# RoboSafe-Lab/Controllable-Latent-Diffusion-for-Traffic-Simulation

Measured on AMD Instinct MI355X. Metric: denoising-step·agent/s, higher is better.
Workload: dtype f32; 1 GPU; BASELINE configs[2]: 32 scenes x 64 agents per GPU, 100 denoising steps (DDPM ancestral loop of the reference), latent seq 52 x 4, cond 256, CFG w=2.0 (2 U-Net passes per step, non_cond_feat); target-speed guidance gradient through decoder + roll-out on every step t > 0; + LSTM decode + unicycle roll-out; scenes_total=32, agents_this_rank=2048, agents_total=2048, denoise_steps=100, guidance_gradient=True, sim_steps_per_bench_step=0, weights=random init (synth seed 0)

## Files before the change

### controllable-latent-diffusion-for-traffic-simulation_amd/csrc/cld_api.hip

```cpp
#include <hip/hip_runtime.h>

#include <cmath>
#include <cstdio>
#include <cstdlib>
#include <cstring>
#include <map>
#include <string>
#include <vector>

#include "../../include/cld.h"
#include "cld_kernels.h"
#include "train.h"

using namespace cld;

namespace {

constexpr int T = 52, D = 4, COND = 256, TE = 32, NCB = 1792, ACT = 3328;
constexpr int NBUF = 8;

struct ConvLayer {
    ConvGeom g{};
    bool has_a = false, has_b = false;
    float *wfrag = nullptr, *bias = nullptr, *gamma = nullptr, *beta = nullptr;
// ... 241 lines not shown
        static const char* th = getenv("CLD_TILING_HALF");
#else
        constexpr const char* th = nullptr;
#endif
        const long wgs_b = (long)(b_pad / (MT / l.g.lm)) * (l.c_out / 32);
        int best = 0;
        double best_cost = 1e30;
        for (int hm = 0; hm <= 3; ++hm) {
            ConvGeom tg = *g; tg.half = hm;
            if (!conv_geom_supported(tg)) continue;
            if (th && th[0] != '0' + hm && (th[0] == '0' || th[0] == '1' || th[0] == '2' || th[0] == '3')) continue;
            const long n = wgs_b << hm, rounds = (n + 255) / 256;
            const int nmt = ((208 >> hm) + 15) / 16;
            double cost = (double)rounds * nmt / (rounds == 1 ? 0.85 : 0.92);
            if (l.g.stride == 2 && hm == 0) cost *= 1.15;
            if (cost < best_cost * (b_pad >= 1024 ? 0.97 : 1.0)) { best_cost = cost; best = hm; }
        }
        if (cost_c <= best_cost) return set(32, 4, 2);
        g->half = best;
        if (best == 3 && (wgs_b << 3) * roles <= 256 && c1c2_mult_of_64(l)) {
            ConvGeom d = *g; d.kc = 64; d.nwn = 2; d.ks = 4;
            if (conv_geom_supported(d)) return set(64, 2, 4);
        }
        return true;
    }
    return false;
}

struct Ws {
    float *xw, *xtmp, *meanb, *cb, *buf[NBUF], *guide;
    float *gcur, *adam_m, *adam_v;
    float *col_traj, *col_grad;
    float* col_act;
};
size_t ws_floats(int b_pad) {
    return (size_t)b_pad * (3 * T * D + NCB + (size_t)NBUF * ACT) + guide_scratch_floats(b_pad) + (size_t)b_pad * (3 * T * D + 2 * T * 6 + T * 2);
}
Ws carve(void* ws, int b_pad) {
    Ws w;
    float* p = static_cast<float*>(ws);
    w.xw = p; p += (size_t)b_pad * T * D;
    w.xtmp = p; p += (size_t)b_pad * T * D;
    w.meanb = p; p += (size_t)b_pad * T * D;
    w.cb = p; p += (size_t)b_pad * NCB;
    for (int i = 0; i < NBUF; ++i) { w.buf[i] = p; p += (size_t)b_pad * ACT; }
    w.guide = p; p += guide_scratch_floats(b_pad);
    w.gcur = p; p += (size_t)b_pad * T * D;
    w.adam_m = p; p += (size_t)b_pad * T * D;
    w.adam_v = p; p += (size_t)b_pad * T * D;
    w.col_traj = p; p += (size_t)b_pad * T * 6;
    w.col_grad = p; p += (size_t)b_pad * T * 6;
    w.col_act = p;
    return w;
}
inline int pad16(int b) { return (b + 15) / 16 * 16; }

ConvArgs make_args(cld_handle h, const ConvLayer& l, const float* x1, const float* x2, float* y, const float* res,
                   const float* cb, const float* tb_row) {
    ConvArgs a{};
    a.x1 = x1; a.x2 = x2; a.c1_real = l.c1_real; a.c1_pad = l.c1_pad; a.c2 = l.c2;
    a.wfrag = l.wfrag; a.bias = l.bias; a.gamma = l.gamma; a.beta = l.beta;
    if (l.cb_off >= 0) { a.cbias = cb + l.cb_off; a.cb_stride = NCB; a.tbias = tb_row ? tb_row + l.cb_off : nullptr; }
    a.res = res; a.y = y; a.c_out = l.c_out; a.ly = l.ly; a.off0 = l.off0; a.orow0 = l.orow0;
    a.wscale_inv = l.g.ain == 1 ? 1.0f / kWScale : 1.0f;
    a.stamps = nullptr;
    (void)h;
    return a;
}

constexpr int kWino1dMinRows = 384;
bool conv5_takes_winograd(int l_in, int c1, int c2, int c_out, long b_pad, int forced) {
    if (!wino1d_supported(l_in, c1, c2, c_out) || forced == CLD_FORM_DIRECT) return false;
    const long widest = c1 > c_out ? c1 : c_out;
    if (b_pad * l_in * widest * 4 >= (1L << 31)) return false;
    return forced == CLD_FORM_WINOGRAD || forced == CLD_FORM_WINOGRAD_WHOLE || forced == CLD_FORM_WINOGRAD_KSPLIT || b_pad >= kWino1dMinRows;
}
int wino_item_form(cld_handle h) {
    const int f = h->force_kernel[CLD_KERNEL_CONV5];
    return f == CLD_FORM_WINOGRAD_WHOLE ? 1 : f == CLD_FORM_WINOGRAD_KSPLIT ? 2 : 0;
}
bool use_wino1d(cld_handle h, const ConvLayer& l, int b_pad) {
    if (!l.ufrag || !l.wino_launch) return false;
    return conv5_takes_winograd(l.g.l_in, l.c1_real, l.c2, l.c_out, b_pad, h->force_kernel[CLD_KERNEL_CONV5]);
}
void count_flop(cld_handle h, const ConvLayer& l, int b_pad, double* alg, double* exec) {
// ... 983 lines not shown
    a.urgency = g->urgency; a.pref_speed = g->pref_speed; a.scale = g->scale; a.reached = g->reached; a.grad_in = grad_in;
    a.loss = loss; a.grad = grad; a.rows = B; a.num_samp = g->num_samp; a.global_t = g->global_t; a.dt = g->dt;
    a.min_progress_dist = g->min_progress_dist;
    return a;
}

static int check_guidance(cld_handle h, const char* fn, const cld_guidance* gd, int B) {
    if (!h->has_decoder) return fail(h, CLD_ERR_STATE, std::string(fn) + ": guidance needs the decoder weights");
    if (!gd->curr_states || (!gd->target_speed && !gd->speed_limit_scale && !gd->acc_limit_scale && !gd->target_pos_scale && !gd->ext_grad && !gd->collision && !gd->map_collision && !h->has_goal))
        return fail(h, CLD_ERR_ARG, std::string(fn) + ": guidance needs curr_states and at least one loss term");
    if (gd->collision) {
        const int rcc = check_collision(h, fn, gd->collision, B);
        if (rcc) return rcc;
    }
    if (gd->map_collision) {
        const int rcc = check_map_collision(h, fn, gd->map_collision, B);
        if (rcc) return rcc;
    }
    if (h->has_goal) {
        const int rcc = check_goal(h, fn, &h->goal, B);
        if (rcc) return rcc;
    }
    if (gd->grad_steps < 0 || gd->final_grad_steps < 0 || gd->grad_steps > 64 || gd->final_grad_steps > 64)
        return fail(h, CLD_ERR_ARG, std::string(fn) + ": grad_steps out of range (0..64)");
    if (gd->optimizer != CLD_GUIDE_ADAM && gd->optimizer != CLD_GUIDE_SGD) return fail(h, CLD_ERR_ARG, std::string(fn) + ": unknown optimizer");
    if (gd->apply_output && gd->final_optimizer != CLD_GUIDE_ADAM && gd->final_optimizer != CLD_GUIDE_SGD)
        return fail(h, CLD_ERR_ARG, std::string(fn) + ": unknown optimizer for the output step");
    if (gd->target_pos_scale && (!gd->target_pos || !gd->target_time)) return fail(h, CLD_ERR_ARG, std::string(fn) + ": target_pos_scale needs target_pos and target_time");
    return CLD_OK;
}

static int run_guidance(cld_handle h, const Ws& w, const cld_guidance* gd, int B, bool intermediate, float sigma_t, float sigma_noise,
                        const float* mean0, const float* cond, const float* z, uint64_t seed, unsigned long long salt,
                        float* mean_out, float* x_out, float* x_out2, float* grad_out, hipStream_t s) {
    GuideArgs g{};
    g.cond = cond; g.curr_states = gd->curr_states; g.target_speed = gd->target_speed; g.loss_scale = gd->loss_scale;
    g.speed_limit_scale = gd->speed_limit_scale; g.acc_limit_scale = gd->acc_limit_scale;
    g.speed_limit = gd->speed_limit; g.acc_limit = gd->acc_limit;
    g.target_pos = gd->target_pos; g.target_time = gd->target_time; g.target_pos_scale = gd->target_pos_scale;
    g.ext_grad = gd->ext_grad;
    const float lr_in = intermediate ? gd->lr : gd->final_lr, th_in = intermediate ? gd->perturb_th : gd->final_perturb_th;
    g.scratch = w.guide; g.lr = lr_in > 0.f ? lr_in : sigma_t; g.perturb_th = th_in > 0.f ? th_in : (th_in == 0.f ? sigma_t : -1.f);
    g.optimizer = intermediate ? gd->optimizer : gd->final_optimizer; g.B = B; g.seed = seed; g.step_salt = salt;
    const int steps_in = intermediate ? gd->grad_steps : gd->final_grad_steps;
    const int steps = steps_in > 1 ? steps_in : 1;
    g.opt_steps = steps; g.mean0 = mean0; g.adam_m = w.adam_m; g.adam_v = w.adam_v;
    for (int k = 1; k <= steps; ++k) {
        const bool last = k == steps;
        g.opt_step = k;
        g.mean = k == 1 ? mean0 : w.gcur;
        if (gd->collision || gd->map_collision || h->has_goal) {
            if (B >= 256 && guide_forward_available(B, h->force_kernel[CLD_KERNEL_GUIDE]) && h->force_kernel[CLD_KERNEL_DECODE] == FORM_AUTO) {
                GuideArgs gf{};
                gf.mean = g.mean; gf.cond = cond; gf.curr_states = gd->curr_states; gf.scratch = w.guide; gf.B = B; gf.act_out = w.col_act;
                HIPCK(h, launch_guide_forward(h->dec, h->dyn, gf, s));
                HIPCK(h, launch_action_to_state(h->dyn, w.col_act, gd->curr_states, w.col_traj, B, 1, 1, s));
                g.act_in = guide_split_available(B, h->force_kernel[CLD_KERNEL_GUIDE]) && h->force_kernel[CLD_KERNEL_GUIDE] == FORM_AUTO ? w.col_act : nullptr;
            } else {
                HIPCK(h, launch_decode(h->dec, h->dyn, g.mean, cond, gd->curr_states, nullptr, w.col_traj, B, 1, s, h->force_kernel[CLD_KERNEL_DECODE]));
            }
        }
        if (gd->collision) {
            const cld_collision* c = gd->collision;
            CollisionArgs ca{};
            ca.traj = w.col_traj; ca.extent = c->extent; ca.world_from_agent = c->world_from_agent; ca.curr_speed = c->curr_speed;
            ca.scene_start = c->scene_start; ca.scene_weight = c->scene_weight; ca.guided = c->guided; ca.excluded = c->excluded; ca.max_scene_agents = c->max_scene_agents; ca.grad_in = gd->ext_grad;
            ca.grad = w.col_grad; ca.B_agents = B / c->num_samp; ca.num_scenes = c->num_scenes; ca.num_samp = c->num_samp;
            ca.num_disks = c->num_disks; ca.buffer_dist = c->buffer_dist; ca.decay_rate = c->decay_rate; ca.moving_speed_th = c->moving_speed_th;
            HIPCK(h, launch_agent_collision(ca, s));
            g.ext_grad = w.col_grad;
        }
        if (gd->map_collision) {
            HIPCK(h, launch_map_collision(map_args(gd->map_collision, w.col_traj, gd->collision ? w.col_grad : gd->ext_grad, nullptr, w.col_grad), B, s));
            g.ext_grad = w.col_grad;
        }
        if (h->has_goal) {
            HIPCK(h, launch_goal(goal_args(&h->goal, w.col_traj, (gd->collision || gd->map_collision) ? w.col_grad : gd->ext_grad, nullptr, w.col_grad, B), s));
            g.ext_grad = w.col_grad;
        }
        g.z = last ? z : nullptr;
        g.sigma = last ? sigma_noise : 0.f;
        g.mean_out = last ? mean_out : w.gcur;
        g.x_out = last ? x_out : nullptr;
        g.x_out2 = last ? x_out2 : nullptr;
        g.grad_out = k == 1 ? grad_out : nullptr;
        HIPCK(h, launch_guide(h->dec, h->dyn, g, s, h->force_kernel[CLD_KERNEL_GUIDE]));
    }
    return CLD_OK;
}

static int sample_iteration(cld_handle h, const Ws& w, bool cfg, int B, int bp, int i, const float* z, uint64_t seed,
                            unsigned long long salt, const float* cond, float guidance_w, const cld_guidance* gd,
                            float* mean_guided, float* grad, bool want_mean, hipStream_t s) {
    const int bpn = cfg ? 2 * bp : bp;
    float* x_hi = w.xw + (size_t)bp * T * D;
    const float sigma = std::exp(0.5f * h->plvc[i]);
    const bool guide = gd && (i > 0 ? !gd->no_intermediate : gd->apply_output != 0);
    HeadArgs a{};
    a.w = h->head_w; a.b = h->head_b; a.x = w.xw; a.B = B; a.b_pad = bp;
    a.z = z;
    a.seed = seed; a.step_salt = salt;
    a.xc = h->x_t_cof[i]; a.nc = h->noise_cof[i];
    a.sg = (i == 0) ? 0.f : sigma;
    if (guide) {
        a.mean_out = w.meanb;
        if (gd->guide_clean) {
            a.xc = h->sqrt_recip_acp[i]; a.nc = h->sqrt_recipm1_acp[i];
        }
    } else {
        a.x_out = w.xw;
        a.x_out2 = cfg ? x_hi : nullptr;
        a.mean_out = (i == 0 || want_mean) ? w.meanb : nullptr;
    }
    h->fuse_upd = cfg ? nullptr : &a;
    const hipError_t eu = run_unet(h, w, w.xw, i, bpn, s);
    h->fuse_upd = nullptr;
    HIPCK(h, eu);
    if (!h->upd_fused) {
        head_source(h, w, a);
        if (cfg) {
            if (a.eps_in) a.eps_in_uncond = a.eps_in + (size_t)bp * T * D;
            else a.f_uncond = w.buf[7] + (size_t)bp * T * 64;
            a.cfg_w = guidance_w;
        }
        HIPCK(h, launch_head(a, s));
    }
    if (guide) {
        int rcg = run_guidance(h, w, gd, B, i > 0, sigma, a.sg, w.meanb, cond, a.z, seed, salt, mean_guided ? mean_guided : (i == 0 ? w.xtmp : nullptr),
                               w.xw, cfg ? x_hi : nullptr, grad, s);
        if (rcg) return rcg;
    }
    return CLD_OK;
}

static int sample_impl(cld_handle h, const char* fn, const float* x_T, const float* noise, const float* cond,
                       const float* non_cond, float guidance_w, const cld_guidance* gd, int32_t steps, float* x0, float* x1,
                       float* logp, int32_t B, uint64_t seed, void* workspace, size_t workspace_bytes, void* stream) {
    const bool cfg = non_cond != nullptr;
    int rc = check_common(h, fn, cfg ? 2 * pad16(B) : B, 0, workspace, workspace_bytes);
    if (rc) return rc;
    if (!x_T || !cond) return fail(h, CLD_ERR_ARG, std::string(fn) + ": null pointer");
    if (steps != loop_steps(h))
        return fail(h, CLD_ERR_ARG, std::string(fn) + ": steps must equal len(range(0, n_timesteps, stride)) = " + std::to_string(loop_steps(h)));
    if (gd && (rc = check_guidance(h, fn, gd, B)) != CLD_OK) return rc;
    hipStream_t s = static_cast<hipStream_t>(stream);
    const int bp = pad16(B), bpn = cfg ? 2 * bp : bp;
    Ws w = carve(workspace, bpn);
    float* x_hi = w.xw + (size_t)bp * T * D;
    HIPCK(h, launch_pack_latent(x_T, w.xw, B, bp, s));
    HIPCK(h, launch_cond_bias(cond, h->wc, h->cbias_b, w.cb, B, bp, NCB, s));
    if (cfg) {
        HIPCK(h, launch_pack_latent(x_T, x_hi, B, bp, s));
        HIPCK(h, launch_cond_bias(non_cond, h->wc, h->cbias_b, w.cb + (size_t)bp * NCB, B, bp, NCB, s));
    }
    for (int it = 0; it < steps; ++it) {
        const int i = (steps - 1 - it) * h->stride;
        rc = sample_iteration(h, w, cfg, B, bp, i, noise ? noise + (size_t)it * B * T * D : nullptr, seed, (unsigned long long)it, cond,
                              guidance_w, gd, nullptr, nullptr, false, s);
        if (rc) return rc;
        if (i == 1 && x1) HIPCK(h, launch_unpack(w.xw, x1, B, s));
        if (i == 0) {
            if (x0) HIPCK(h, launch_unpack(w.xw, x0, B, s));
            if (logp) HIPCK(h, launch_logprob(w.xw, (gd && gd->apply_output) ? w.xtmp : w.meanb, std::exp(0.5f * h->plvc[0]), logp, B, s));
        }
    }
    return CLD_OK;
}

int cld_sample_step(cld_handle h, const float* x_t, const float* cond, const float* non_cond, float guidance_w,
                    const cld_guidance* gd, int32_t t_idx, const float* z, float* x_next, float* mean, float* mean_guided,
                    float* grad, float* sigma_host, int32_t B, void* workspace, size_t workspace_bytes, void* stream) {
    const bool cfg = non_cond != nullptr;
    int rc = check_common(h, "cld_sample_step", cfg ? 2 * pad16(B) : B, t_idx, workspace, workspace_bytes);
    if (rc) return rc;
    if (!x_t || !cond || (!z && t_idx != 0)) return fail(h, CLD_ERR_ARG, "cld_sample_step: null pointer");
    if (gd && (rc = check_guidance(h, "cld_sample_step", gd, B)) != CLD_OK) return rc;
    if (sigma_host) *sigma_host = std::exp(0.5f * h->plvc[t_idx]);
    hipStream_t s = static_cast<hipStream_t>(stream);
    const int bp = pad16(B), bpn = cfg ? 2 * bp : bp;
    Ws w = carve(workspace, bpn);
    HIPCK(h, launch_pack_latent(x_t, w.xw, B, bp, s));
    HIPCK(h, launch_cond_bias(cond, h->wc, h->cbias_b, w.cb, B, bp, NCB, s));
    if (cfg) {
        HIPCK(h, launch_pack_latent(x_t, w.xw + (size_t)bp * T * D, B, bp, s));
        HIPCK(h, launch_cond_bias(non_cond, h->wc, h->cbias_b, w.cb + (size_t)bp * NCB, B, bp, NCB, s));
    }
    rc = sample_iteration(h, w, cfg, B, bp, t_idx, z, 0, 0, cond, guidance_w, gd, mean_guided, grad, mean != nullptr, s);
    if (rc) return rc;
    if (x_next) HIPCK(h, launch_unpack(w.xw, x_next, B, s));
    if (mean) HIPCK(h, launch_unpack(w.meanb, mean, B, s));
    return CLD_OK;
// ... 461 lines not shown
```

### controllable-latent-diffusion-for-traffic-simulation_amd/csrc/cld_kernels.h

```cpp
#pragma once
#include <hip/hip_runtime.h>
#include <stdint.h>

namespace cld {

inline hipError_t set_max_lds_once(const void* fn, int bytes, unsigned long long* done_mask) {
    int dev = 0;
    hipError_t e = hipGetDevice(&dev);
    if (e != hipSuccess) return e;
    if (dev >= 0 && dev < 64 && ((*done_mask >> dev) & 1ull)) return hipSuccess;
    e = hipFuncSetAttribute(fn, hipFuncAttributeMaxDynamicSharedMemorySize, bytes);
    if (e != hipSuccess) return e;
    if (dev >= 0 && dev < 64) *done_mask |= 1ull << dev;
    return hipSuccess;
}

constexpr int MT = 208;
constexpr int NMT = 13;

enum { EPI_BIAS = 0, EPI_GN_MISH = 1 };

struct ConvArgs {
    const float* x1;
    const float* x2;
// ... 203 lines not shown
    const float *c_wt[5], *c_b[5], *c_g[4], *c_be[4];
};
hipError_t launch_context_head(const ContextHeadArgs& a, hipStream_t s);

struct GuideArgs {
    const float* mean;
    const float* cond;
    const float* curr_states;
    const float* target_speed;
    const float* loss_scale;
    const float* speed_limit_scale;
    const float* acc_limit_scale;
    float speed_limit, acc_limit;
    const float* target_pos;
    const int* target_time;
    const float* target_pos_scale;
    const float* ext_grad;
    const float* z;
    float* mean_out;
    float* x_out;
    float* x_out2;
    float* grad_out;
    float* act_out;
    const float* act_in;
    float* scratch;
    float lr, perturb_th, sigma;
    int optimizer;
    int opt_step, opt_steps;
    const float* mean0;
    float* adam_m;
    float* adam_v;
    int B;
    unsigned long long seed, step_salt;
};
size_t guide_scratch_floats(int B);
void read_guide_stamps(unsigned long long* out);
hipError_t launch_guide(const DecoderWeights& w, const DynParams& d, const GuideArgs& a, hipStream_t s, int form = FORM_AUTO);
bool guide_forward_available(int B, int form = FORM_AUTO);
bool guide_split_available(int B, int form = FORM_AUTO);
hipError_t launch_guide_forward(const DecoderWeights& w, const DynParams& d, const GuideArgs& a, hipStream_t s);

hipError_t launch_guide_losses(const GuideArgs& a, const float* traj, float* losses, hipStream_t s);

struct CollisionArgs {
    const float* traj;
    const float* extent;
    const float* world_from_agent;
    const float* curr_speed;
    const int* scene_start;
    const float* scene_weight;
    const unsigned char* guided;
    const unsigned char* excluded;
    const float* grad_in;
    float* loss;
    float* grad;
    int B_agents, num_scenes, num_samp, num_disks;
    int max_scene_agents;
    float buffer_dist, decay_rate, moving_speed_th;
};
hipError_t launch_agent_collision(const CollisionArgs& a, hipStream_t s);

struct MapCollisionArgs {
    const float* traj;
    const float* extent;
    const float* raster_from_agent;
    const unsigned char* drivable_map;
    const float* curr_speed;
    const int* scene_start;
// ... 64 lines not shown
```

### controllable-latent-diffusion-for-traffic-simulation_amd/csrc/guide_kernels.hip

```cpp
#include "cld_kernels.h"

namespace cld {

typedef float v4f __attribute__((ext_vector_type(4)));

__device__ __forceinline__ float sigmoid_g(float x) { return 1.0f / (1.0f + expf(-x)); }

constexpr int GT = 52;
__device__ __forceinline__ void chain_grad(const DynParams& d, const GuideArgs& a, int b, const float* act0, const float* act1, int st,
                                           float* dact0, float* dact1, float* sc) {
    float* vk = sc; float* th = sc + 54; float* gv = sc + 108; float* gth = sc + 162;
    float* gxk = sc + 216; float* gyk = sc + 270;
    const float* cs = a.curr_states + (size_t)b * 4;
    const float* tgt = a.target_speed ? a.target_speed + (size_t)b * GT : nullptr;
    const float s_ts = tgt ? (a.loss_scale ? a.loss_scale[b] : (1.0f / (float)GT)) : 0.f;
    const float s_sl = a.speed_limit_scale ? a.speed_limit_scale[b] : 0.f;
    const float s_al = a.acc_limit_scale ? a.acc_limit_scale[b] : 0.f;
    const float s_tp = a.target_pos_scale ? a.target_pos_scale[b] : 0.f;
    const float* eg = a.ext_grad ? a.ext_grad + (size_t)b * GT * 6 : nullptr;
    const bool pos = s_tp != 0.f || eg != nullptr;
    float v_raw = cs[2], x = cs[0], y = cs[1], yaw = cs[3];
    vk[0] = fminf(fmaxf(v_raw, d.v_lo), d.v_hi);
    th[0] = yaw;
    gv[0] = 0.f;
// ... 969 lines not shown

__device__ __forceinline__ float sum_over_units(float x) {
    x += __builtin_bit_cast(float, __builtin_amdgcn_update_dpp(0, __builtin_bit_cast(int, x), 0x124 , 0xf, 0xf, false));
    x += __builtin_bit_cast(float, __builtin_amdgcn_update_dpp(0, __builtin_bit_cast(int, x), 0x128 , 0xf, 0xf, false));
    const auto r16 = __builtin_amdgcn_permlane16_swap(__builtin_bit_cast(unsigned, x), __builtin_bit_cast(unsigned, x), false, false);
    const unsigned a16 = r16[0], b16 = r16[1];
    x = __builtin_bit_cast(float, a16) + __builtin_bit_cast(float, b16);
    const auto r32 = __builtin_amdgcn_permlane32_swap(__builtin_bit_cast(unsigned, x), __builtin_bit_cast(unsigned, x), false, false);
    const unsigned a32 = r32[0], b32 = r32[1];
    return __builtin_bit_cast(float, a32) + __builtin_bit_cast(float, b32);
}

__device__ __forceinline__ float add_other_half(float x) {
    const auto r32 = __builtin_amdgcn_permlane32_swap(__builtin_bit_cast(unsigned, x), __builtin_bit_cast(unsigned, x), false, false);
    const unsigned a32 = r32[0], b32 = r32[1];
    return __builtin_bit_cast(float, a32) + __builtin_bit_cast(float, b32);
}

__device__ __forceinline__ float quad_xor1(float v) { return __builtin_bit_cast(float, __builtin_amdgcn_update_dpp(0, __builtin_bit_cast(int, v), 0xB1 , 0xf, 0xf, false)); }
__device__ __forceinline__ float quad_xor2(float v) { return __builtin_bit_cast(float, __builtin_amdgcn_update_dpp(0, __builtin_bit_cast(int, v), 0x4E , 0xf, 0xf, false)); }
__device__ __forceinline__ v4f quad_transpose(const v4f& x, bool odd1, bool odd2) {
    const float x0 = x[0], x1 = x[1], x2 = x[2], x3 = x[3];
    const float r01 = quad_xor1(odd1 ? x0 : x1), r23 = quad_xor1(odd1 ? x2 : x3);
    const float y0 = odd1 ? r01 : x0, y1 = odd1 ? x1 : r01, y2 = odd1 ? r23 : x2, y3 = odd1 ? x3 : r23;
    const float r02 = quad_xor2(odd2 ? y0 : y2), r13 = quad_xor2(odd2 ? y1 : y3);
    return v4f{odd2 ? r02 : y0, odd2 ? r13 : y1, odd2 ? y2 : r02, odd2 ? y3 : r13};
}

namespace gq {
constexpr int AG = 8, HS = 80, GS = 272;
constexpr int ACTS = GT * 2 * 5 * 512;
}

__global__ __launch_bounds__(512) void guide_quad_kernel(const DecoderWeights w, const DynParams d, const GuideArgs a) {
    using namespace gq;
    __shared__ __attribute__((aligned(16))) float hs[2][2][AG][HS];
    __shared__ __attribute__((aligned(16))) float dG[2][AG][GS];
    __shared__ __attribute__((aligned(16))) float zin[AG][208];
    __shared__ __attribute__((aligned(16))) float condm[AG][256];
    __shared__ __attribute__((aligned(16))) float hpart[4][AG][HS];
    __shared__ __attribute__((aligned(16))) float xch[2][8][64][4];
    __shared__ float actp[GT][2][4][AG];
    __shared__ float act[2][GT][AG];
    __shared__ float dact[AG][2][GT];
    __shared__ float chs[AG][CG_ROWS * 54];
    __shared__ float dz[AG][208];
    const int tid = threadIdx.x, lane = tid & 63;
    const int wv8 = __builtin_amdgcn_readfirstlane(tid >> 6);
    const int wq = wv8 & 3, kp = wv8 >> 2;
    const int ul = lane >> 2, q = lane & 3;
    const int u = 16 * wq + ul;
    const int ao = 4 * kp + q;
    const float wa0 = w.w_h2a[u], wa1 = w.w_h2a[64 + u], bh2a = w.b_h2a[0], bh2b = w.b_h2a[1];

    const int ngroups = (a.B + AG - 1) / AG;
    for (int grp = blockIdx.x; grp < ngroups; grp += gridDim.x) {
        const int b0 = grp * AG;
        GSTAMP(0);
        const __amdgpu_buffer_rsrc_t keep = __builtin_amdgcn_make_buffer_rsrc(a.scratch + (size_t)blockIdx.x * ACTS, 0, ACTS * 4, 0x00020000);
        const int kvo = tid * 4;
        auto kput = [&](int slot, float v) { __builtin_amdgcn_raw_buffer_store_b32(__builtin_bit_cast(unsigned, v), keep, kvo, slot * 2048, 0); };
        auto kget = [&](int slot) { return __builtin_bit_cast(float, __builtin_amdgcn_raw_buffer_load_b32(keep, kvo, slot * 2048, 0)); };
        auto agent = [&](int ag) { return (b0 + ag < a.B) ? b0 + ag : a.B - 1; };
        for (int i = tid; i < AG * 256; i += 512) condm[i >> 8][i & 255] = a.cond[(size_t)agent(i >> 8) * 256 + (i & 255)];
        for (int i = tid; i < AG * 208; i += 512) zin[i / 208][i % 208] = a.mean[(size_t)agent(i / 208) * 208 + i % 208];
        __syncthreads();
        const bool backward_only = a.act_in != nullptr;
        float c0 = 0.f, c1 = 0.f;
        GPHASE_DECL;
        if (!backward_only) {
        if (wv8 < 4) {
            const float* wr = w.w_c2h + (size_t)(4 * ul + q) * 256 + 64 * wv8;
            asm volatile("" : "+v"(wr));
            v4f p0 = {0.f, 0.f, 0.f, 0.f}, p1 = p0, p2 = p0, p3 = p0;
#pragma unroll
            for (int j = 0; j < 16; ++j) {
                const v4f wa = *reinterpret_cast<const v4f*>(wr + 4 * j);
                const v4f ca = *reinterpret_cast<const v4f*>(&condm[q][64 * wv8 + 4 * j]);
                const v4f cb = *reinterpret_cast<const v4f*>(&condm[4 + q][64 * wv8 + 4 * j]);
#pragma unroll
                for (int e = 0; e < 4; e += 2) {
                    p0 = CLD_MFMA4(wa[e], ca[e], p0); p1 = CLD_MFMA4(wa[e], cb[e], p1);
                    p2 = CLD_MFMA4(wa[e + 1], ca[e + 1], p2); p3 = CLD_MFMA4(wa[e + 1], cb[e + 1], p3);
                }
            }
#pragma unroll
            for (int r = 0; r < 4; ++r) {
                hpart[wv8][q][4 * ul + r] = p0[r] + p2[r];
                hpart[wv8][4 + q][4 * ul + r] = p1[r] + p3[r];
            }
        }
        __syncthreads();
        {
            const int ag = tid >> 6, uu = tid & 63;
            const float v = w.b_c2h[uu] + hpart[0][ag][uu] + hpart[1][ag][uu] + hpart[2][ag][uu] + hpart[3][ag][uu];
            hs[0][0][ag][uu] = v;
            hs[1][0][ag][uu] = v;
        }
        __syncthreads();
        GSTAMP(1);
        {
            const size_t row = (size_t)(64 * q + u);
            const float *p0a = w.w_ih0 + row * 4, *p0b = w.w_hh0 + row * 64 + 32 * kp, *p1 = (kp ? w.w_hh1 : w.w_ih1) + row * 64, *p_b0 = w.b0 + u, *p_b1 = w.b1 + u;
            asm volatile("" : "+v"(p0a), "+v"(p0b), "+v"(p1), "+v"(p_b0), "+v"(p_b1));
            v4f W0[9], W1[16];
            W0[0] = *reinterpret_cast<const v4f*>(p0a);
            if (kp) W0[0] = v4f{0.f, 0.f, 0.f, 0.f};
#pragma unroll
            for (int j = 0; j < 8; ++j) W0[1 + j] = *reinterpret_cast<const v4f*>(p0b + 4 * j);
#pragma unroll
            for (int j = 0; j < 16; ++j) W1[j] = *reinterpret_cast<const v4f*>(p1 + 4 * j);
            const float bq0 = kp ? 0.f : p_b0[64 * q], bq1 = kp ? 0.f : p_b1[64 * q];
            const v4f bias0 = {bq0, bq0, bq0, bq0}, bias1 = {bq1, bq1, bq1, bq1};
            const v4f zero = {0.f, 0.f, 0.f, 0.f};
            v4f keep0, keep1;
            auto half0 = [&](int t) {
                const int pr = t & 1;
                const v4f Xx[2] = {*reinterpret_cast<const v4f*>(&zin[q][4 * t]), *reinterpret_cast<const v4f*>(&zin[4 + q][4 * t])};
                const v4f Xh[2] = {*reinterpret_cast<const v4f*>(&hs[0][pr][q][32 * kp + 4 * (ul & 7)]), *reinterpret_cast<const v4f*>(&hs[0][pr][4 + q][32 * kp + 4 * (ul & 7)])};
                v4f a00 = bias0, a01 = zero, a10 = bias0, a11 = zero;
                bsweep<0, 1, 4>(&Xx[0], &Xx[1], [&](int) { return W0[0]; }, a00, a01, a10, a11);
                bsweep<0, 8, 4>(&Xh[0], &Xh[1], [&](int g) { return W0[1 + g]; }, a00, a01, a10, a11);
                const v4f P0 = a00 + a01, P1 = a10 + a11;
                *reinterpret_cast<v4f*>(&xch[0][wv8][lane][0]) = kp ? P0 : P1;
                keep0 = kp ? P1 : P0;
            };
            auto half1 = [&](int t) {
                const float* src = &hs[0][0][0][0] + (kp ? 2 * AG * HS + (t & 1) * AG * HS : ((t & 1) ^ 1) * AG * HS);
                const v4f X[2] = {*reinterpret_cast<const v4f*>(src + q * HS + 4 * ul), *reinterpret_cast<const v4f*>(src + (4 + q) * HS + 4 * ul)};
                v4f a00 = bias1, a01 = zero, a10 = bias1, a11 = zero;
                bsweep<0, 16, 4>(&X[0], &X[1], [&](int g) { return W1[g]; }, a00, a01, a10, a11);
                const v4f P0 = a00 + a01, P1 = a10 + a11;
                *reinterpret_cast<v4f*>(&xch[1][wv8][lane][0]) = kp ? P0 : P1;
                keep1 = kp ? P1 : P0;
            };
            auto cell0 = [&](int t) {
                const v4f P = quad_transpose(keep0 + *reinterpret_cast<const v4f*>(&xch[0][wv8 ^ 4][lane][0]), q & 1, q & 2);
                const float i_ = fsig(P[0]), f_ = fsig(P[1]), g_ = ftanh(P[2]), o_ = fsig(P[3]);
                const float c = f_ * c0 + i_ * g_;
                c0 = c;
                hs[0][(t & 1) ^ 1][ao][u] = o_ * ftanh(c);
                const int ks = (t * 2 + 0) * 5;
                kput(ks + 0, i_); kput(ks + 1, f_); kput(ks + 2, g_); kput(ks + 3, o_); kput(ks + 4, c);
            };
            auto cell1 = [&](int t) {
// ... 24 lines not shown
                lds_barrier();
                GPHASE(2);
                if (t + 2 < GT) half0(t + 2);
                GPHASE(3);
                if (t + 1 < GT) half1(t + 1);
                GPHASE(4);
                lds_barrier();
                GPHASE(5);
            }
        }
        GSTAMP(3);
        for (int i = tid; i < 2 * GT * AG; i += 512) {
            const int o = i / (GT * AG), t = (i / AG) % GT, ag = i % AG;
            act[o][t][ag] = (o ? bh2b : bh2a) + actp[t][o][0][ag] + actp[t][o][1][ag] + actp[t][o][2][ag] + actp[t][o][3][ag];
        }
        } else {
            for (int i = tid; i < 2 * GT * AG; i += 512) {
                const int ag = i / (2 * GT), t = (i >> 1) % GT, o = i & 1;
                act[o][t][ag] = a.act_in[((size_t)agent(ag) * GT + t) * 2 + o];
            }
        }
        __syncthreads();
        if (a.act_out) {
            for (int i = tid; i < 2 * GT * AG; i += 512) {
                const int ag = i / (2 * GT), t = (i >> 1) % GT, o = i & 1;
                if (b0 + ag < a.B) a.act_out[((size_t)(b0 + ag) * GT + t) * 2 + o] = act[o][t][ag];
            }
            __syncthreads();
            continue;
        }
        chain_grad_group<AG, 512>(d, a, agent, &act[0][0][0], &act[1][0][0], AG, &dact[0][0][0], &chs[0][0]);
        GSTAMP(4);
        {
            const v4f* gf = reinterpret_cast<const v4f*>(w.gqfrag) + (size_t)wq * (2 * 32 * 64) + (size_t)kp * (16 * 64) + lane;
            asm volatile("" : "+v"(gf));
            v4f t1[16], t0[16];
#pragma unroll
            for (int j = 0; j < 16; ++j) { t1[j] = gf[j * 64]; t0[j] = gf[(32 + j) * 64]; }
            const int kh = lane >> 5;
            const int src_rec = ul * 4, src_dwn = src_rec + 64, rsel = q;
            auto pick = [&](const v4f& v, int byte_lane) {
                const float x0 = bperm(byte_lane, v[0]), x1 = bperm(byte_lane, v[1]), x2 = bperm(byte_lane, v[2]), x3 = bperm(byte_lane, v[3]);
                return rsel == 0 ? x0 : (rsel == 1 ? x1 : (rsel == 2 ? x2 : x3));
            };
            v4f keepS1 = {0.f, 0.f, 0.f, 0.f}, keepS0 = keepS1;
            auto halfprod = [&](int lay, const v4f (&tw)[16], v4f& keepS) {
                const float* gq0 = &dG[lay][q][128 * kh + 64 * kp + 4 * (ul & 7)];
                const float* gq1 = &dG[lay][4 + q][128 * kh + 64 * kp + 4 * (ul & 7)];
                const v4f X0[2] = {*reinterpret_cast<const v4f*>(gq0), *reinterpret_cast<const v4f*>(gq0 + 32)};
                const v4f X1[2] = {*reinterpret_cast<const v4f*>(gq1), *reinterpret_cast<const v4f*>(gq1 + 32)};
                v4f p00 = {0.f, 0.f, 0.f, 0.f}, p01 = p00, p10 = p00, p11 = p00;
                bsweep<0, 16, 3>(X0, X1, [&](int g) { return tw[g]; }, p00, p01, p10, p11);
                v4f S0 = p00 + p01, S1 = p10 + p11;
#pragma unroll
                for (int r = 0; r < 4; ++r) { S0[r] = add_other_half(S0[r]); S1[r] = add_other_half(S1[r]); }
                *reinterpret_cast<v4f*>(&xch[lay][wv8][lane][0]) = kp ? S0 : S1;
                keepS = kp ? S1 : S0;
            };
            float rec1 = 0.f, rec0 = 0.f, down = 0.f, dc1n = 0.f, dc0n = 0.f;
            float kv1[6], kv0[6];
            auto fetch = [&](float (&kv)[6], int t, int layer) {
                const int ks = (t * 2 + layer) * 5;
#pragma unroll
                for (int k = 0; k < 5; ++k) kv[k] = kget(ks + k);
                kv[5] = t > 0 ? kget(ks - 10 + 4) : 0.f;
            };
            auto grads = [&](const float (&kv)[6], float dh, float& dcn, float* row) {
                const float i_ = kv[0], f_ = kv[1], g_ = kv[2], o_ = kv[3], c = kv[4], cp = kv[5];
// ... 66 lines not shown
                if (a.sigma != 0.f) zz = a.z ? a.z[(size_t)b * 208 + r] : normal4(a.seed, a.step_salt, (unsigned)(b * 52 + (r >> 2)))[r & 3];
                const float xn = mu + a.sigma * zz;
                a.x_out[(size_t)b * 208 + r] = xn;
                if (a.x_out2) a.x_out2[(size_t)b * 208 + r] = xn;
            }
        }
        __syncthreads();
    }
}

static int guide_mfma_grid(int B) {
    const int groups = (B + gm8::AG - 1) / gm8::AG;
    return groups < 256 ? groups : 256;
}
static int guide_quad_grid(int B) {
    const int groups = (B + gq::AG - 1) / gq::AG;
    return groups < 256 ? groups : 256;
}
static int guide_form(int B, int form) {
    if (form != FORM_AUTO) return form;
    if (B < 64) return FORM_VALU;
    const int r8 = (B + 8 * 256 - 1) / (8 * 256), r16 = (B + 16 * 256 - 1) / (16 * 256);
    return 2 * r8 < 3 * r16 ? FORM_MFMA_QUAD : FORM_MFMA;
}
size_t guide_scratch_floats(int B) {
    const size_t valu = (size_t)guide_grid(B) * GNA * (G_GATES + G_CELLS);
    const size_t mfma = (size_t)guide_mfma_grid(B) * gm8::ACTS, quad = (size_t)guide_quad_grid(B) * gq::ACTS;
    return valu > mfma ? (valu > quad ? valu : quad) : (mfma > quad ? mfma : quad);
}

bool guide_forward_available(int B, int form) { return guide_form(B, form) == FORM_MFMA_QUAD; }
bool guide_split_available(int B, int form) { return guide_form(B, form) == FORM_MFMA_QUAD && (B + gq::AG - 1) / gq::AG <= guide_quad_grid(B); }
hipError_t launch_guide_forward(const DecoderWeights& w, const DynParams& d, const GuideArgs& a, hipStream_t s) {
    if (!a.act_out || a.act_in) return hipErrorInvalidValue;
    hipLaunchKernelGGL(guide_quad_kernel, dim3(guide_quad_grid(a.B)), dim3(512), 0, s, w, d, a);
    return hipGetLastError();
}

hipError_t launch_guide(const DecoderWeights& w, const DynParams& d, const GuideArgs& a, hipStream_t s, int form) {
    if (a.act_in && !guide_split_available(a.B, form)) return hipErrorInvalidValue;
    switch (guide_form(a.B, form)) {
        case FORM_MFMA_QUAD: hipLaunchKernelGGL(guide_quad_kernel, dim3(guide_quad_grid(a.B)), dim3(512), 0, s, w, d, a); break;
        case FORM_MFMA: hipLaunchKernelGGL(guide_mfma8_kernel, dim3(guide_mfma_grid(a.B)), dim3(512), 0, s, w, d, a); break;
        default: hipLaunchKernelGGL(guide_kernel, dim3(guide_grid(a.B)), dim3(256), 0, s, w, d, a);
    }
    return hipGetLastError();
}

}

namespace cld {

__global__ __launch_bounds__(64) void reward_kernel(const RewardArgs a) {
    const int b = blockIdx.x, t = threadIdx.x;
    float off = 0.f, col = 0.f, jerk = 0.f;
    if (t < 52) {
        const float* p = a.traj + ((size_t)b * 52 + t) * 6;
        const float x = p[0], y = p[1];
        const float* R = a.raster_from_agent + (size_t)b * 9;
        const float rx = x * R[0] + y * R[1] + R[2];
        const float ry = x * R[3] + y * R[4] + R[5];
        long cx = (long)rintf(rx), cy = (long)rintf(ry);
        cx = cx < 0 ? 0 : (cx > a.W - 1 ? a.W - 1 : cx);
        cy = cy < 0 ? 0 : (cy > a.H - 1 ? a.H - 1 : cy);
        off = a.drivable_map[((size_t)b * a.H + cy) * a.W + cx] ? 0.f : -1.f;
        if (t < a.To) {
            for (int s = 0; s < a.S; ++s) {
                const size_t o = ((size_t)b * a.S + s) * a.To + t;
                const float dx = x - a.other_pos[2 * o], dy = y - a.other_pos[2 * o + 1];
                if (sqrtf(dx * dx + dy * dy) < a.collision_thresh && a.other_avail[o]) col -= 1.f;
            }
        }
        if (t < 51 && a.traj_scaled) {
// ... 75 lines not shown
```

Before: 813,100 step·agent/s.

## Fold CFG head into guide kernel and precompute cond-to-hidden once per sample

The cond-to-hidden projection, which depends only on the conditioning, is now computed once before the denoising loop into a workspace buffer and read by the guide kernel instead of being recomputed on every step. When guidance runs without collision, map or goal terms, the classifier-free-guidance head (eps combination and mean update) is folded into the first optimizer step of the guide kernel, removing a separate head launch and a global round trip for the mean. This adds kernel parameters and workspace, and ties head fusion to the quad MFMA guide form.

Result: no change. 815,100 step·agent/s (median of 6 runs) (+0.2%).

```diff
diff --git a/controllable-latent-diffusion-for-traffic-simulation_amd/csrc/cld_api.hip b/controllable-latent-diffusion-for-traffic-simulation_amd/csrc/cld_api.hip
--- a/controllable-latent-diffusion-for-traffic-simulation_amd/csrc/cld_api.hip
+++ b/controllable-latent-diffusion-for-traffic-simulation_amd/csrc/cld_api.hip
@@ -297,9 +297,10 @@
     float *gcur, *adam_m, *adam_v;
     float *col_traj, *col_grad;
     float* col_act;
+    float* h_init;
 };
 size_t ws_floats(int b_pad) {
-    return (size_t)b_pad * (3 * T * D + NCB + (size_t)NBUF * ACT) + guide_scratch_floats(b_pad) + (size_t)b_pad * (3 * T * D + 2 * T * 6 + T * 2);
+    return (size_t)b_pad * (3 * T * D + NCB + (size_t)NBUF * ACT) + guide_scratch_floats(b_pad) + (size_t)b_pad * (3 * T * D + 2 * T * 6 + T * 2 + 64);
 }
 Ws carve(void* ws, int b_pad) {
     Ws w;
@@ -315,7 +316,8 @@
     w.adam_v = p; p += (size_t)b_pad * T * D;
     w.col_traj = p; p += (size_t)b_pad * T * 6;
     w.col_grad = p; p += (size_t)b_pad * T * 6;
-    w.col_act = p;
+    w.col_act = p; p += (size_t)b_pad * T * 2;
+    w.h_init = p;
     return w;
 }
 inline int pad16(int b) { return (b + 15) / 16 * 16; }
@@ -1365,9 +1367,10 @@
 
 static int run_guidance(cld_handle h, const Ws& w, const cld_guidance* gd, int B, bool intermediate, float sigma_t, float sigma_noise,
                         const float* mean0, const float* cond, const float* z, uint64_t seed, unsigned long long salt,
-                        float* mean_out, float* x_out, float* x_out2, float* grad_out, hipStream_t s) {
+                        float* mean_out, float* x_out, float* x_out2, float* grad_out, hipStream_t s,
+                        const float* h_init = nullptr, const HeadArgs* fold = nullptr) {
     GuideArgs g{};
-    g.cond = cond; g.curr_states = gd->curr_states; g.target_speed = gd->target_speed; g.loss_scale = gd->loss_scale;
+    g.cond = cond; g.h_init = h_init; g.curr_states = gd->curr_states; g.target_speed = gd->target_speed; g.loss_scale = gd->loss_scale;
     g.speed_limit_scale = gd->speed_limit_scale; g.acc_limit_scale = gd->acc_limit_scale;
     g.speed_limit = gd->speed_limit; g.acc_limit = gd->acc_limit;
     g.target_pos = gd->target_pos; g.target_time = gd->target_time; g.target_pos_scale = gd->target_pos_scale;
@@ -1382,10 +1385,16 @@
         const bool last = k == steps;
         g.opt_step = k;
         g.mean = k == 1 ? mean0 : w.gcur;
+        if (fold) {
+            const bool first = k == 1;
+            g.head_x = first ? fold->x : nullptr; g.head_eps = fold->eps_in; g.head_eps_uncond = fold->eps_in_uncond;
+            g.head_mean_out = fold->mean_out; g.head_xc = fold->xc; g.head_nc = fold->nc; g.head_cfg_w = fold->cfg_w;
+            g.mean0 = first ? nullptr : mean0;
+        }
         if (gd->collision || gd->map_collision || h->has_goal) {
             if (B >= 256 && guide_forward_available(B, h->force_kernel[CLD_KERNEL_GUIDE]) && h->force_kernel[CLD_KERNEL_DECODE] == FORM_AUTO) {
                 GuideArgs gf{};
-                gf.mean = g.mean; gf.cond = cond; gf.curr_states = gd->curr_states; gf.scratch = w.guide; gf.B = B; gf.act_out = w.col_act;
+                gf.mean = g.mean; gf.cond = cond; gf.curr_states = gd->curr_states; gf.scratch = w.guide; gf.B = B; gf.act_out = w.col_act; gf.h_init = h_init;
                 HIPCK(h, launch_guide_forward(h->dec, h->dyn, gf, s));
                 HIPCK(h, launch_action_to_state(h->dyn, w.col_act, gd->curr_states, w.col_traj, B, 1, 1, s));
                 g.act_in = guide_split_available(B, h->force_kernel[CLD_KERNEL_GUIDE]) && h->force_kernel[CLD_KERNEL_GUIDE] == FORM_AUTO ? w.col_act : nullptr;
@@ -1424,7 +1433,8 @@
 
 static int sample_iteration(cld_handle h, const Ws& w, bool cfg, int B, int bp, int i, const float* z, uint64_t seed,
                             unsigned long long salt, const float* cond, float guidance_w, const cld_guidance* gd,
-                            float* mean_guided, float* grad, bool want_mean, hipStream_t s) {
+                            float* mean_guided, float* grad, bool want_mean, hipStream_t s, const float* h_init = nullptr,
+                            bool fold_head = false) {
     const int bpn = cfg ? 2 * bp : bp;
     float* x_hi = w.xw + (size_t)bp * T * D;
     const float sigma = std::exp(0.5f * h->plvc[i]);
@@ -1449,6 +1459,7 @@
     const hipError_t eu = run_unet(h, w, w.xw, i, bpn, s);
     h->fuse_upd = nullptr;
     HIPCK(h, eu);
+    bool folded = false;
     if (!h->upd_fused) {
         head_source(h, w, a);
         if (cfg) {
@@ -1456,11 +1467,13 @@
             else a.f_uncond = w.buf[7] + (size_t)bp * T * 64;
             a.cfg_w = guidance_w;
         }
-        HIPCK(h, launch_head(a, s));
+        folded = fold_head && guide && cfg && a.eps_in && guide_forward_available(B, h->force_kernel[CLD_KERNEL_GUIDE]) &&
+                 !gd->collision && !gd->map_collision && !h->has_goal;
+        if (!folded) HIPCK(h, launch_head(a, s));
     }
     if (guide) {
         int rcg = run_guidance(h, w, gd, B, i > 0, sigma, a.sg, w.meanb, cond, a.z, seed, salt, mean_guided ? mean_guided : (i == 0 ? w.xtmp : nullptr),
-                               w.xw, cfg ? x_hi : nullptr, grad, s);
+                               w.xw, cfg ? x_hi : nullptr, grad, s, h_init, folded ? &a : nullptr);
         if (rcg) return rcg;
     }
     return CLD_OK;
@@ -1486,10 +1499,15 @@
         HIPCK(h, launch_pack_latent(x_T, x_hi, B, bp, s));
         HIPCK(h, launch_cond_bias(non_cond, h->wc, h->cbias_b, w.cb + (size_t)bp * NCB, B, bp, NCB, s));
     }
+    const float* h_init = nullptr;
+    if (gd && guide_forward_available(B, h->force_kernel[CLD_KERNEL_GUIDE])) {
+        HIPCK(h, launch_cond2hidden(h->dec, cond, w.h_init, B, s));
+        h_init = w.h_init;
+    }
     for (int it = 0; it < steps; ++it) {
         const int i = (steps - 1 - it) * h->stride;
         rc = sample_iteration(h, w, cfg, B, bp, i, noise ? noise + (size_t)it * B * T * D : nullptr, seed, (unsigned long long)it, cond,
-                              guidance_w, gd, nullptr, nullptr, false, s);
+                              guidance_w, gd, nullptr, nullptr, false, s, h_init, true);
         if (rc) return rc;
         if (i == 1 && x1) HIPCK(h, launch_unpack(w.xw, x1, B, s));
         if (i == 0) {
diff --git a/controllable-latent-diffusion-for-traffic-simulation_amd/csrc/cld_kernels.h b/controllable-latent-diffusion-for-traffic-simulation_amd/csrc/cld_kernels.h
--- a/controllable-latent-diffusion-for-traffic-simulation_amd/csrc/cld_kernels.h
+++ b/controllable-latent-diffusion-for-traffic-simulation_amd/csrc/cld_kernels.h
@@ -259,8 +259,15 @@
     float* adam_v;
     int B;
     unsigned long long seed, step_salt;
+    const float* h_init;
+    const float* head_x;
+    const float* head_eps;
+    const float* head_eps_uncond;
+    float* head_mean_out;
+    float head_xc, head_nc, head_cfg_w;
 };
 size_t guide_scratch_floats(int B);
+hipError_t launch_cond2hidden(const DecoderWeights& w, const float* cond, float* h_init, int B, hipStream_t s);
 void read_guide_stamps(unsigned long long* out);
 hipError_t launch_guide(const DecoderWeights& w, const DynParams& d, const GuideArgs& a, hipStream_t s, int form = FORM_AUTO);
 bool guide_forward_available(int B, int form = FORM_AUTO);
diff --git a/controllable-latent-diffusion-for-traffic-simulation_amd/csrc/guide_kernels.hip b/controllable-latent-diffusion-for-traffic-simulation_amd/csrc/guide_kernels.hip
--- a/controllable-latent-diffusion-for-traffic-simulation_amd/csrc/guide_kernels.hip
+++ b/controllable-latent-diffusion-for-traffic-simulation_amd/csrc/guide_kernels.hip
@@ -1025,6 +1025,66 @@
 constexpr int ACTS = GT * 2 * 5 * 512;
 }
 
+__device__ __forceinline__ float cond2hidden8(const DecoderWeights& w, const float (&condm)[gq::AG][256], float (&hpart)[4][gq::AG][gq::HS]) {
+    const int tid = threadIdx.x, lane = tid & 63;
+    const int wv8 = __builtin_amdgcn_readfirstlane(tid >> 6);
+    const int ul = lane >> 2, q = lane & 3;
+    if (wv8 < 4) {
+        int wo = (4 * ul + q) * 256;
+        asm volatile("" : "+v"(wo));
+        const float* wr = w.w_c2h + wo + 64 * wv8;
+        v4f p0 = {0.f, 0.f, 0.f, 0.f}, p1 = p0, p2 = p0, p3 = p0;
+#pragma unroll
+        for (int j = 0; j < 16; ++j) {
+            const v4f wa = *reinterpret_cast<const v4f*>(wr + 4 * j);
+            const v4f ca = *reinterpret_cast<const v4f*>(&condm[q][64 * wv8 + 4 * j]);
+            const v4f cb = *reinterpret_cast<const v4f*>(&condm[4 + q][64 * wv8 + 4 * j]);
+#pragma unroll
+            for (int e = 0; e < 4; e += 2) {
+                p0 = CLD_MFMA4(wa[e], ca[e], p0); p1 = CLD_MFMA4(wa[e], cb[e], p1);
+                p2 = CLD_MFMA4(wa[e + 1], ca[e + 1], p2); p3 = CLD_MFMA4(wa[e + 1], cb[e + 1], p3);
+            }
+        }
+#pragma unroll
+        for (int r = 0; r < 4; ++r) {
+            hpart[wv8][q][4 * ul + r] = p0[r] + p2[r];
+            hpart[wv8][4 + q][4 * ul + r] = p1[r] + p3[r];
+        }
+    }
+    __syncthreads();
+    const int ag = tid >> 6;
+    int uu = tid & 63;
+    asm volatile("" : "+v"(uu));
+    return w.b_c2h[uu] + hpart[0][ag][uu] + hpart[1][ag][uu] + hpart[2][ag][uu] + hpart[3][ag][uu];
+}
+
+__global__ __launch_bounds__(512) void cond2hidden8_kernel(const DecoderWeights w, const float* __restrict__ cond, float* __restrict__ h_init, int B) {
+    using namespace gq;
+    __shared__ __attribute__((aligned(16))) float condm[AG][256];
+    __shared__ __attribute__((aligned(16))) float hpart[4][AG][HS];
+    const int tid = threadIdx.x, b0 = blockIdx.x * AG;
+    for (int i = tid; i < AG * 256; i += 512) {
+        const int b = b0 + (i >> 8);
+        condm[i >> 8][i & 255] = cond[(size_t)(b < B ? b : B - 1) * 256 + (i & 255)];
+    }
+    __syncthreads();
+    const float v = cond2hidden8(w, condm, hpart);
+    if (b0 + (tid >> 6) < B) h_init[(size_t)(b0 + (tid >> 6)) * 64 + (tid & 63)] = v;
+}
+hipError_t launch_cond2hidden(const DecoderWeights& w, const float* cond, float* h_init, int B, hipStream_t s) {
+    hipLaunchKernelGGL(cond2hidden8_kernel, dim3((B + gq::AG - 1) / gq::AG), dim3(512), 0, s, w, cond, h_init, B);
+    return hipGetLastError();
+}
+
+__device__ __forceinline__ float folded_head_mean(const GuideArgs& a, size_t e, int ch) {
+#pragma clang fp contract(off)
+    const float ec = a.head_eps[e], eu = a.head_eps_uncond[e], x = a.head_x[e];
+    const float w1 = 1.0f + a.head_cfg_w, pu = a.head_cfg_w * eu;
+    const float pc = w1 * ec;
+    const float eps = ch < 2 ? fmaf(w1, ec, -pu) : pc - pu;
+    return fmaf(a.head_xc, x, -(a.head_nc * eps));
+}
+
 __global__ __launch_bounds__(512) void guide_quad_kernel(const DecoderWeights w, const DynParams d, const GuideArgs a) {
     using namespace gq;
     __shared__ __attribute__((aligned(16))) float hs[2][2][AG][HS];
@@ -1055,47 +1115,37 @@
         auto kput = [&](int slot, float v) { __builtin_amdgcn_raw_buffer_store_b32(__builtin_bit_cast(unsigned, v), keep, kvo, slot * 2048, 0); };
         auto kget = [&](int slot) { return __builtin_bit_cast(float, __builtin_amdgcn_raw_buffer_load_b32(keep, kvo, slot * 2048, 0)); };
         auto agent = [&](int ag) { return (b0 + ag < a.B) ? b0 + ag : a.B - 1; };
-        for (int i = tid; i < AG * 256; i += 512) condm[i >> 8][i & 255] = a.cond[(size_t)agent(i >> 8) * 256 + (i & 255)];
-        for (int i = tid; i < AG * 208; i += 512) zin[i / 208][i % 208] = a.mean[(size_t)agent(i / 208) * 208 + i % 208];
-        __syncthreads();
         const bool backward_only = a.act_in != nullptr;
+        const bool own_c2h = !backward_only && !a.h_init;
+        if (own_c2h)
+            for (int i = tid; i < AG * 256; i += 512) condm[i >> 8][i & 255] = a.cond[(size_t)agent(i >> 8) * 256 + (i & 255)];
+        if (a.head_x) {
+            for (int i = tid; i < AG * 208; i += 512) {
+                const int ag = i / 208, r = i % 208;
+                const size_t e = (size_t)agent(ag) * 208 + r;
+                const float m = folded_head_mean(a, e, r & 3);
+                zin[ag][r] = m;
+                if (b0 + ag < a.B) a.head_mean_out[e] = m;
+            }
+        } else {
+            for (int i = tid; i < AG * 208; i += 512) zin[i / 208][i % 208] = a.mean[(size_t)agent(i / 208) * 208 + i % 208];
+        }
+        __syncthreads();
         float c0 = 0.f, c1 = 0.f;
         GPHASE_DECL;
         if (!backward_only) {
-        if (wv8 < 4) {
-            const float* wr = w.w_c2h + (size_t)(4 * ul + q) * 256 + 64 * wv8;
-            asm volatile("" : "+v"(wr));
-            v4f p0 = {0.f, 0.f, 0.f, 0.f}, p1 = p0, p2 = p0, p3 = p0;
-#pragma unroll
-            for (int j = 0; j < 16; ++j) {
-                const v4f wa = *reinterpret_cast<const v4f*>(wr + 4 * j);
-                const v4f ca = *reinterpret_cast<const v4f*>(&condm[q][64 * wv8 + 4 * j]);
-                const v4f cb = *reinterpret_cast<const v4f*>(&condm[4 + q][64 * wv8 + 4 * j]);
-#pragma unroll
-                for (int e = 0; e < 4; e += 2) {
-                    p0 = CLD_MFMA4(wa[e], ca[e], p0); p1 = CLD_MFMA4(wa[e], cb[e], p1);
-                    p2 = CLD_MFMA4(wa[e + 1], ca[e + 1], p2); p3 = CLD_MFMA4(wa[e + 1], cb[e + 1], p3);
-                }
-            }
-#pragma unroll
-            for (int r = 0; r < 4; ++r) {
-                hpart[wv8][q][4 * ul + r] = p0[r] + p2[r];
-                hpart[wv8][4 + q][4 * ul + r] = p1[r] + p3[r];
-            }
-        }
-        __syncthreads();
         {
             const int ag = tid >> 6, uu = tid & 63;
-            const float v = w.b_c2h[uu] + hpart[0][ag][uu] + hpart[1][ag][uu] + hpart[2][ag][uu] + hpart[3][ag][uu];
+            const float v = own_c2h ? cond2hidden8(w, condm, hpart) : a.h_init[(size_t)agent(ag) * 64 + uu];
             hs[0][0][ag][uu] = v;
             hs[1][0][ag][uu] = v;
         }
         __syncthreads();
         GSTAMP(1);
         {
-            const size_t row = (size_t)(64 * q + u);
-            const float *p0a = w.w_ih0 + row * 4, *p0b = w.w_hh0 + row * 64 + 32 * kp, *p1 = (kp ? w.w_hh1 : w.w_ih1) + row * 64, *p_b0 = w.b0 + u, *p_b1 = w.b1 + u;
-            asm volatile("" : "+v"(p0a), "+v"(p0b), "+v"(p1), "+v"(p_b0), "+v"(p_b1));
+            int row = 64 * q + u;
+            asm volatile("" : "+v"(row));
+            const float *p0a = w.w_ih0 + row * 4, *p0b = w.w_hh0 + row * 64 + 32 * kp, *p1 = (kp ? w.w_hh1 : w.w_ih1) + row * 64;
             v4f W0[9], W1[16];
             W0[0] = *reinterpret_cast<const v4f*>(p0a);
             if (kp) W0[0] = v4f{0.f, 0.f, 0.f, 0.f};
@@ -1103,7 +1153,7 @@
             for (int j = 0; j < 8; ++j) W0[1 + j] = *reinterpret_cast<const v4f*>(p0b + 4 * j);
 #pragma unroll
             for (int j = 0; j < 16; ++j) W1[j] = *reinterpret_cast<const v4f*>(p1 + 4 * j);
-            const float bq0 = kp ? 0.f : p_b0[64 * q], bq1 = kp ? 0.f : p_b1[64 * q];
+            const float bq0 = kp ? 0.f : w.b0[row], bq1 = kp ? 0.f : w.b1[row];
             const v4f bias0 = {bq0, bq0, bq0, bq0}, bias1 = {bq1, bq1, bq1, bq1};
             const v4f zero = {0.f, 0.f, 0.f, 0.f};
             v4f keep0, keep1;
@@ -1194,8 +1244,9 @@
         chain_grad_group<AG, 512>(d, a, agent, &act[0][0][0], &act[1][0][0], AG, &dact[0][0][0], &chs[0][0]);
         GSTAMP(4);
         {
-            const v4f* gf = reinterpret_cast<const v4f*>(w.gqfrag) + (size_t)wq * (2 * 32 * 64) + (size_t)kp * (16 * 64) + lane;
-            asm volatile("" : "+v"(gf));
+            int gl = lane;
+            asm volatile("" : "+v"(gl));
+            const v4f* gf = reinterpret_cast<const v4f*>(w.gqfrag) + (size_t)wq * (2 * 32 * 64) + (size_t)kp * (16 * 64) + gl;
             v4f t1[16], t0[16];
 #pragma unroll
             for (int j = 0; j < 16; ++j) { t1[j] = gf[j * 64]; t0[j] = gf[(32 + j) * 64]; }
@@ -1328,13 +1379,14 @@
 bool guide_forward_available(int B, int form) { return guide_form(B, form) == FORM_MFMA_QUAD; }
 bool guide_split_available(int B, int form) { return guide_form(B, form) == FORM_MFMA_QUAD && (B + gq::AG - 1) / gq::AG <= guide_quad_grid(B); }
 hipError_t launch_guide_forward(const DecoderWeights& w, const DynParams& d, const GuideArgs& a, hipStream_t s) {
-    if (!a.act_out || a.act_in) return hipErrorInvalidValue;
+    if (!a.act_out || a.act_in || a.head_x) return hipErrorInvalidValue;
     hipLaunchKernelGGL(guide_quad_kernel, dim3(guide_quad_grid(a.B)), dim3(512), 0, s, w, d, a);
     return hipGetLastError();
 }
 
 hipError_t launch_guide(const DecoderWeights& w, const DynParams& d, const GuideArgs& a, hipStream_t s, int form) {
     if (a.act_in && !guide_split_available(a.B, form)) return hipErrorInvalidValue;
+    if (a.head_x && (guide_form(a.B, form) != FORM_MFMA_QUAD || !a.head_eps || !a.head_eps_uncond || !a.head_mean_out)) return hipErrorInvalidValue;
     switch (guide_form(a.B, form)) {
         case FORM_MFMA_QUAD: hipLaunchKernelGGL(guide_quad_kernel, dim3(guide_quad_grid(a.B)), dim3(512), 0, s, w, d, a); break;
         case FORM_MFMA: hipLaunchKernelGGL(guide_mfma8_kernel, dim3(guide_mfma_grid(a.B)), dim3(512), 0, s, w, d, a); break;
```
